# yanx27/PointASNL

Hardware: AMD Instinct MI355X
Metric: point-clouds/sec fwd (Bx1024 pts, ModelNet40 cls) (higher is better)
Workload: dtype f32; 1 GPU; configs[1]: ModelNet40 pointasnl_cls, 1024 pts, batch=64/GPU, seeded random weights; global_batch=64, parallelism=batch-shard x1, RCCL all-gather of logits, pipeline=prefetch, hip_graph=True, prefix_forked_at=start, prefix_levels=2, settle_replays=40, hip_hw_queues=4

## Files before the change

### include/pasnl.h

```cpp
#ifndef PASNL_H_
#define PASNL_H_

#include <stddef.h>
#include <stdint.h>

#ifdef __cplusplus
extern "C" {
#endif

#define PASNL_VERSION 100

enum {
  PASNL_OK = 0,
  PASNL_EINVAL = -1,
  PASNL_ENULL = -2,
  PASNL_EWORKSPACE = -3,
  PASNL_ELAUNCH = -4,
  PASNL_EUNSUPPORTED = -5
};

typedef void* pasnl_stream_t;

int pasnl_version(void);
const char* pasnl_strerror(int code);
// ... 90 lines not shown
                          const float* ww, const float* bw, float* out, float* skip_max, float* new_xyz, float* new_feature,
                          pasnl_stream_t stream);

int pasnl_sa_project(int b, int n, int c, int c1, const float* xyz, const float* feature, const float* w0, const float* b0,
                     float* proj, pasnl_stream_t stream);
int pasnl_sa_cell_pre(int b, int n, int c, int m, int k, int c1, int c2, const float* xyz, const float* feature,
                      const float* proj, const int* idx, const float* new_xyz, const float* w0, const float* w1, const float* b1,
                      const float* ww, const float* bw, float* out, float* skip_max, pasnl_stream_t stream);
int pasnl_sa_cell_pre_centre0(int b, int n, int c, int m, int k, int c1, int c2, const float* xyz, const float* feature,
                              const float* proj, const int* idx, const float* w0, const float* w1, const float* b1,
                              const float* ww, const float* bw, float* out, float* skip_max, float* new_xyz, float* new_feature,
                              pasnl_stream_t stream);

int pasnl_sa_cell_packed(int b, int n, int c, int npoint, int nsample, int c1, int c2, const float* xyz, const float* feature,
                         const int* idx, const float* new_xyz, const float* w0, const float* b0, const float* w1, const float* b1,
                         const float* ww, const float* bw, const float* w0_features_packed, const float* w1_packed, float* out,
                         float* skip_max, float* new_xyz_out, float* new_feature_out, pasnl_stream_t stream);

int pasnl_max_pool_rows(int b, int n, int c, const float* x, float* out, pasnl_stream_t stream);

int pasnl_max_pool_rows_strided(int b, int n, int c, const float* x, float* out, long out_stride, pasnl_stream_t stream);

size_t pasnl_mlp3_packed_weights_bytes(int k, int n);
int pasnl_mlp3_pack_weights(int k, int n, const float* w, float* packed, pasnl_stream_t stream);
size_t pasnl_mlp3_max_pool_workspace_bytes(int b, int n, int c3);
int pasnl_mlp3_max_pool(int b, int n, int k0, int c1, int c2, int c3, const float* x, const float* w0, const float* b0,
                        const float* w1, const float* b1, const float* w2, const float* b2, float* out, long out_stride,
                        void* workspace, size_t workspace_bytes, pasnl_stream_t stream);

int pasnl_cls_tail_group_all(int b, int n, int w, int cb, int c, const float* after, const float* skip_max, const float* att,
                             const float* ws_packed, const float* bs, const float* wb_packed, const float* bb,
                             const float* wagg_packed, const float* bagg, const float* new_xyz, int c1, int c2, int c3,
                             const float* w0, const float* b0, const float* w1, const float* b1, const float* w2, const float* b2,
                             float* out, float* pooled, long pooled_stride, void* workspace, size_t workspace_bytes,
                             pasnl_stream_t stream);

size_t pasnl_bf16x3_weights_bytes(int kdim, int n);
int pasnl_bf16x3_split_weights(int kdim, int n, const float* w, void* wsplit, pasnl_stream_t stream);
int pasnl_dense_bf16x3(int rows, int kdim, int n, int lda, const float* x, const void* wsplit, const float* bias, int relu,
                       float* out, pasnl_stream_t stream);


size_t pasnl_dense_rows_workspace_bytes(int rows, int kdim, int n);
int pasnl_dense_rows(int rows, int kdim, int n, const float* x, const float* w, const float* bias, int relu, float* out,
                     void* workspace, size_t workspace_bytes, pasnl_stream_t stream);

size_t pasnl_dense_splitk_workspace_bytes(int rows, int kdim, int n);
int pasnl_dense_splitk(int rows, int kdim, int n, int lda, const float* x, const float* w, const float* bias, int relu,
                       float* out, void* workspace, size_t workspace_bytes, pasnl_stream_t stream);

int pasnl_narrow_project2(long rows0, int kdim0, int n0, const float* x0, const float* w0, const float* bias0, float* out0,
                          long rows1, int kdim1, int n1, const float* x1, const float* w1, const float* bias1, float* out1,
                          pasnl_stream_t stream);

size_t pasnl_grad_workspace_bytes(int b, int targets, long contributions);
int pasnl_gather_point_grad_det(int b, int n, int m, const float* out_g, const int* idx, float* inp_g, void* workspace,
                                size_t workspace_bytes, pasnl_stream_t stream);
int pasnl_group_point_grad_det(int b, int n, int c, int m, int nsample, const float* grad_out, const int* idx,
                               float* grad_points, void* workspace, size_t workspace_bytes, pasnl_stream_t stream);
int pasnl_three_interpolate_grad_det(int b, int n, int c, int m, const float* grad_out, const int* idx, const float* weight,
                                     float* grad_points, void* workspace, size_t workspace_bytes, pasnl_stream_t stream);

int pasnl_sa_tail(int rows, int w, int cb, int c, const float* after, const float* skip_max, const float* att, const float* ws,
                  const float* bs, const float* wb, const float* bb, const float* wagg, const float* bagg, float* out,
                  pasnl_stream_t stream);

int pasnl_sa_tail_res(int rows, int w, int cb, int c, const float* after, const float* skip_max, const float* att,
                      const float* ws, const float* bs, const float* wb, const float* bb, const float* wagg,
                      const float* bagg, const float* residual, float* out, pasnl_stream_t stream);

size_t pasnl_sa_tail_packed_weights_bytes(int k, int c);
int pasnl_sa_tail_pack_weights(int k, int c, const float* w, float* packed, pasnl_stream_t stream);
int pasnl_sa_tail_packed(int rows, int w, int cb, int c, const float* after, const float* skip_max, const float* att,
                         const float* ws_packed, const float* bs, const float* wb_packed, const float* bb, const float* wagg_packed,
                         const float* bagg, const float* residual, const float* new_xyz, float* out_cat, float* out,
                         pasnl_stream_t stream);

int pasnl_sa_tail_cat(int rows, int w, int cb, int c, const float* after, const float* skip_max, const float* att,
                      const float* ws, const float* bs, const float* wb, const float* bb, const float* wagg,
                      const float* bagg, float* out, const float* new_xyz, float* out_cat, pasnl_stream_t stream);

int pasnl_decode_cell(int b, int n, int c, int k, const float* xyz, const float* feature, const int* idx, const float* ww,
                      const float* bw, float* out, pasnl_stream_t stream);

int pasnl_decode_cell_tiled(int b, int n, int c, int k, const float* xyz, const float* feature, const int* idx,
                            const float* ww, const float* bw, float* out, pasnl_stream_t stream);
int pasnl_decode_cell_tiled_v4(int c, const float* feature);

int pasnl_take_neighbor0(int b, int n, int c, int m, int k, const float* xyz, const float* feature, const int* idx,
                         float* new_xyz, float* new_feature, pasnl_stream_t stream);

int pasnl_as_gather(int b, int n, int c, int m, int k, int as, const float* xyz, const float* feature, const int* idx, float* out,
                    pasnl_stream_t stream);
int pasnl_as_attention_qkv(int g, int as, int cb, const float* kvq, float* out, pasnl_stream_t stream);
int pasnl_as_attention_proj(int g, int as, int cb, int w, const float* x, const float* wkvq, const float* bkvq, float* out,
                            pasnl_stream_t stream);
int pasnl_as_cell_narrow(int g, int as, int cb, int w, int ch, const float* x, const float* wkvq, const float* bkvq,
                         const float* wa, const float* ba, const float* wb, const float* bb, float* new_xyz, float* new_feature,
                         pasnl_stream_t stream);
int pasnl_as_cell_wide(int g, int as, int cb, int w, int ch, const float* kvq, const float* x, const float* wa, const float* ba,
                       const float* wb, const float* bb, float* new_xyz, float* new_feature, pasnl_stream_t stream);

int pasnl_as_cell_wide_ld(int g, int as, int cb, int w, int ch, const float* kvq, int ld, const float* x, const float* wa,
                          const float* ba, const float* wb, const float* bb, float* new_xyz, float* new_feature,
                          pasnl_stream_t stream);
int pasnl_as_reweight_x(int g, int as, int ch, const float* logits, const float* x, float* new_xyz, float* new_feature,
// ... 223 lines not shown
```

### pointasnl_amd/_hip.py

```python
import ctypes
import os

import torch

_HERE = os.path.dirname(os.path.abspath(__file__))
LIB_PATH = os.path.join(_HERE, "csrc", "libpasnl_hip.so")

SYMBOLS = [
    "pasnl_version", "pasnl_strerror", "pasnl_device_count",
    "pasnl_farthest_point_sample", "pasnl_farthest_point_sample_gather", "pasnl_gather_point", "pasnl_gather_point_grad", "pasnl_prob_sample",
    "pasnl_query_ball_point", "pasnl_sa_group", "pasnl_group_point", "pasnl_group_point_grad", "pasnl_select_top_k", "pasnl_knn_batch", "pasnl_knn_workspace_bytes", "pasnl_knn_batch_ws", "pasnl_knn_batch_ws_bg", "pasnl_knn_tree_workspace_bytes", "pasnl_knn_batch_tree", "pasnl_knn_batch_ref_workspace_bytes", "pasnl_knn_batch_ref", "pasnl_knn_distance_pick",
    "pasnl_three_nn", "pasnl_three_interpolate", "pasnl_three_interpolate_grad", "pasnl_three_weights", "pasnl_fp_interpolate_cat",
    "pasnl_nl_attention", "pasnl_nl_attention_workspace_bytes", "pasnl_nl_attention_ws", "pasnl_as_attention", "pasnl_as_reweight", "pasnl_sa_local_cell", "pasnl_sa_cell", "pasnl_sa_cell_centre0", "pasnl_sa_cell_packed", "pasnl_sa_project", "pasnl_sa_cell_pre", "pasnl_sa_cell_pre_centre0", "pasnl_sa_tail", "pasnl_sa_tail_cat", "pasnl_sa_tail_res", "pasnl_sa_tail_packed_weights_bytes", "pasnl_sa_tail_pack_weights", "pasnl_sa_tail_packed", "pasnl_decode_cell", "pasnl_decode_cell_tiled", "pasnl_decode_cell_tiled_v4", "pasnl_max_pool_rows", "pasnl_max_pool_rows_strided", "pasnl_mlp3_max_pool_workspace_bytes", "pasnl_mlp3_max_pool", "pasnl_mlp3_packed_weights_bytes", "pasnl_mlp3_pack_weights", "pasnl_dense_rows_workspace_bytes", "pasnl_dense_rows", "pasnl_dense_splitk_workspace_bytes", "pasnl_dense_splitk", "pasnl_bf16x3_weights_bytes", "pasnl_bf16x3_split_weights", "pasnl_dense_bf16x3", "pasnl_narrow_project2", "pasnl_take_neighbor0", "pasnl_as_gather", "pasnl_as_attention_qkv", "pasnl_as_attention_proj", "pasnl_as_cell_narrow", "pasnl_as_cell_wide", "pasnl_as_cell_wide_ld", "pasnl_as_reweight_x", "pasnl_grid_subsample_workspace_bytes", "pasnl_grid_subsample", "pasnl_knn_crop_workspace_bytes", "pasnl_knn_crop",
    "pasnl_scan_pick", "pasnl_knn_crop_indirect", "pasnl_crop_order_permute", "pasnl_scan_possibility_update", "pasnl_scan_scratch_init", "pasnl_scan_vote", "pasnl_scan_reproject_workspace_bytes", "pasnl_scan_reproject", "pasnl_scan_labels",
    "pasnl_scan_pick_given", "pasnl_scan_train_labels", "pasnl_scan_augment",
    "pasnl_scan_radius_workspace_bytes", "pasnl_scan_radius_members", "pasnl_scene_radius_members", "pasnl_scan_radius_gather", "pasnl_scene_radius_gather",
    "pasnl_scene_pick", "pasnl_knn_crop_scene", "pasnl_scene_pick_crop", "pasnl_scene_order_gather", "pasnl_scene_potential_update", "pasnl_scene_vote", "pasnl_scene_labels", "pasnl_confusion_matrix",
    "pasnl_window_noise", "pasnl_window_bounds", "pasnl_window_hist_bytes", "pasnl_window_count", "pasnl_window_fill", "pasnl_window_gather", "pasnl_window_vote", "pasnl_window_pool_labels",
    "pasnl_kwindow_hist_bytes", "pasnl_kwindow_count", "pasnl_kwindow_fill", "pasnl_kwindow_gather",
    "pasnl_modelnet_fps_cap", "pasnl_modelnet_fps", "pasnl_modelnet_normalize", "pasnl_modelnet_batch", "pasnl_modelnet_augment", "pasnl_modelnet_noise", "pasnl_cls_vote", "pasnl_cls_tally",
    "pasnl_cls_tail_group_all",
    "pasnl_block_key_capacity", "pasnl_block_crop_stats", "pasnl_block_grid_count", "pasnl_block_fill", "pasnl_block_gather", "pasnl_block_normalize", "pasnl_block_score_workspace_bytes", "pasnl_block_score", "pasnl_block_train_batch", "pasnl_block_train_score",
    "pasnl_kblock_crop_stats", "pasnl_kblock_grid_count", "pasnl_kblock_fill", "pasnl_kblock_gather", "pasnl_kblock_rotate",
    "pasnl_grad_workspace_bytes", "pasnl_gather_point_grad_det", "pasnl_group_point_grad_det", "pasnl_three_interpolate_grad_det",
]


class PasnlError(RuntimeError):
    pass


class PasnlUnsupported(PasnlError):
    """PASNL_EUNSUPPORTED: a valid request outside what the fused kernel covers (include/pasnl.h documents the limits).
    The cells catch it and take their op-by-op path (still HIP kernels + vendor GEMMs, never a CPU path)."""


_lib = None


def lib():
    global _lib
    if _lib is None:
        if not os.path.exists(LIB_PATH):
            raise PasnlError(
                f"{LIB_PATH} is missing: build it with `python -c 'import __graft_entry__ as g; g.build()'` "
                "(or `make -C pointasnl_amd/csrc`).  pointasnl_amd has no CPU or eager fallback.")
        _lib = ctypes.CDLL(LIB_PATH)
        _lib.pasnl_strerror.restype = ctypes.c_char_p
        _lib.pasnl_grad_workspace_bytes.restype = ctypes.c_size_t
        _lib.pasnl_knn_workspace_bytes.restype = ctypes.c_size_t
        _lib.pasnl_knn_tree_workspace_bytes.restype = ctypes.c_size_t
        _lib.pasnl_knn_batch_ref_workspace_bytes.restype = ctypes.c_size_t
        _lib.pasnl_dense_rows_workspace_bytes.restype = ctypes.c_size_t
        _lib.pasnl_bf16x3_weights_bytes.restype = ctypes.c_size_t
        _lib.pasnl_mlp3_max_pool_workspace_bytes.restype = ctypes.c_size_t
        _lib.pasnl_mlp3_packed_weights_bytes.restype = ctypes.c_size_t
        _lib.pasnl_sa_tail_packed_weights_bytes.restype = ctypes.c_size_t
        _lib.pasnl_dense_splitk_workspace_bytes.restype = ctypes.c_size_t
        _lib.pasnl_grid_subsample_workspace_bytes.restype = ctypes.c_size_t
        _lib.pasnl_knn_crop_workspace_bytes.restype = ctypes.c_size_t
        _lib.pasnl_scan_reproject_workspace_bytes.restype = ctypes.c_size_t
        _lib.pasnl_scan_radius_workspace_bytes.restype = ctypes.c_size_t
        _lib.pasnl_nl_attention_workspace_bytes.restype = ctypes.c_size_t
        _lib.pasnl_window_hist_bytes.restype = ctypes.c_size_t
        _lib.pasnl_kwindow_hist_bytes.restype = ctypes.c_size_t
        _lib.pasnl_block_score_workspace_bytes.restype = ctypes.c_size_t
        for s in SYMBOLS:
            getattr(_lib, s)
    return _lib


def require_device():
    if not torch.cuda.is_available():
        raise PasnlError("no HIP device visible: pointasnl_amd runs on MI355X (gfx950) only and has no CPU fallback")
# ... 99 lines not shown
```

### pointasnl_amd/models/pointasnl_cls.py

```python
import torch

from pointasnl_amd.utils import tf_util, pointasnl_util
from pointasnl_amd.utils.pointnet_util import pointnet_sa_module
from pointasnl_amd.utils.pointasnl_util import PointASNLSetAbstraction, get_repulsion_loss, sa_search, Forked


def first_layer(num_point=None):
    return dict(npoint=512, nsample=32)


def get_model(point_cloud, is_training=False, use_normal=False, bn_decay=None, weight_decay=None, num_class=40,
              adaptive_sample=False, search=None, before_head=None, fork_at="head", lazy_fork=None):
    if lazy_fork is None:
        lazy_fork = not adaptive_sample
    batch_size = point_cloud.shape[0]
    end_points = {}
    if use_normal:
        l0_xyz = point_cloud[:, :, 0:3].contiguous()
        l0_points = point_cloud[:, :, 3:6].contiguous()
    else:
        l0_xyz = point_cloud
        l0_points = point_cloud
    end_points['l0_xyz'] = l0_xyz
    as_neighbor = [12, 12] if adaptive_sample else [0, 0]

    net = torch.empty((batch_size, 1024 + 512), dtype=torch.float32, device=point_cloud.device)
    fuse3_1 = not adaptive_sample or pointasnl_util.SA_TAIL_GROUP_ALL == "always"

    search2 = []
    if isinstance(search, dict):
        search2.append(search[2])
        search = search[1]
    l1_xyz, l1_points = PointASNLSetAbstraction(l0_xyz, l0_points, npoint=512, nsample=32, mlp=[64, 64, 128],
                                                is_training=is_training, bn_decay=bn_decay, weight_decay=weight_decay,
                                                scope='layer1', as_neighbor=as_neighbor[0], search=search, xyz_concat=True,
                                                group_all=dict(mlp=[128, 256, 512], scope='layer3_1', pooled_out=net[:, 1024:]) if fuse3_1 else None,
                                                after_sampling=None if search2 else lambda xyz1: search2.append(
                                                    Forked(lambda: sa_search(xyz1, None, 128, 64), lazy=lazy_fork)))
    end_points['l1_xyz'] = l1_xyz
    l2_xyz, l2_points = PointASNLSetAbstraction(l1_xyz, l1_points, npoint=128, nsample=64, mlp=[128, 128, 256],
                                                is_training=is_training, bn_decay=bn_decay, weight_decay=weight_decay,
                                                scope='layer2', as_neighbor=as_neighbor[1], search=search2[0], xyz_concat=True,
                                                after_cell=before_head if fork_at == "cell2" else None,
                                                before_after_conv=before_head if fork_at == "conv2" else None)
    end_points['l2_xyz'] = l1_xyz
    if before_head is not None and fork_at == "head":
        before_head()
    if getattr(l1_points, "group_all_pooled", None) is None:
        _, l3_points_res, _ = pointnet_sa_module(l1_xyz, l1_points, npoint=None, radius=None, nsample=None,
                                                 mlp=[128, 256, 512], mlp2=None, group_all=True, is_training=is_training,
                                                 bn_decay=bn_decay, scope='layer3_1', pooled_out=net[:, 1024:])
    _, l3_points, _ = pointnet_sa_module(l2_xyz, l2_points, npoint=None, radius=None, nsample=None,
                                         mlp=[256, 512, 1024], mlp2=None, group_all=True, is_training=is_training,
                                         bn_decay=bn_decay, scope='layer3_2', pooled_out=net[:, :1024])

    net = tf_util.fully_connected(net, 512, bn=True, is_training=is_training, scope='fc1', bn_decay=bn_decay)
    net = tf_util.dropout(net, keep_prob=0.4, is_training=is_training, scope='dp1')
    net = tf_util.fully_connected(net, 256, bn=True, is_training=is_training, scope='fc2', bn_decay=bn_decay)
    net = tf_util.dropout(net, keep_prob=0.4, is_training=is_training, scope='dp2')
    net = tf_util.fully_connected(net, num_class, activation_fn=None, scope='fc3')
    end_points['l1_points'] = l1_points
    end_points['l2_points'] = l2_points
    end_points['l2_xyz_true'] = l2_xyz
    return net, end_points


def get_loss(pred, label, end_points, uniform_weight=0, weights_decay=1e-4):
    regularization_loss = tf_util.regularization_loss(weights_decay)
    loss = torch.nn.functional.cross_entropy(pred, label.long(), reduction='none')
    classify_loss = loss.mean()
    if uniform_weight > 0:
        uniform_loss = get_repulsion_loss(end_points['l1_xyz'], nsample=20, radius=0.07)
    else:
        uniform_loss = classify_loss
    return classify_loss + uniform_weight * uniform_loss + regularization_loss
```

### pointasnl_amd/utils/pointasnl_util.py

```python

import ctypes

import torch

from pointasnl_amd import _hip
from pointasnl_amd import tf_sampling, tf_grouping, nearest_neighbors
from pointasnl_amd.tf_interpolate import three_nn, three_interpolate, three_weights, fp_interpolate_cat
from pointasnl_amd.utils import tf_util, pointnet_util

NL_KEY_PARTS = True
NL_VARIANT = 0


KNN_TIE_ORDER = "reference"


def knn_query(k, support_pts, query_pts, out=None, max_workgroups=None):
    return nearest_neighbors.knn_batch(support_pts, query_pts, k, omp=True, dtype=torch.int32, tie_order=KNN_TIE_ORDER, out=out,
                                       max_workgroups=max_workgroups)


def _gather_rows(points, idx):
    return tf_grouping.group_point(points, idx.unsqueeze(-1)).squeeze(2)

# ... 302 lines not shown
            with tf_util.variable_scope('mlp2_1'):
                wb, bb = st.layer(32, 1 + channel, bn, weight_decay)
            ld = (3 * cb + 31) // 32 * 32 if AS_PAD_PROJECTION else 3 * cb
            if ld != 3 * cb:
                pkey = key + "@ld%d" % ld
                if pkey not in st._folded:
                    st._folded[pkey] = (torch.cat([wkvq, wkvq.new_zeros((6 + c, ld - 3 * cb))], dim=1).contiguous(),
                                        torch.cat([bkvq, bkvq.new_zeros(ld - 3 * cb)]).contiguous())
                wkvq, bkvq = st._folded[pkey]
            kvq = torch.addmm(bkvq, x.reshape(-1, 6 + c), wkvq)
            new_xyz = torch.empty((b, p, 3), dtype=torch.float32, device=xyz.device)
            new_feature = torch.empty((b, p, channel), dtype=torch.float32, device=xyz.device)
            _hip.launch("pasnl_as_cell_wide_ld", "as_cell", b * p, as_, cb, 6 + c, channel, _hip.ptr(kvq), int(ld), _hip.ptr(x),
                        _hip.ptr(wa), _hip.ptr(ba), _hip.ptr(wb), _hip.ptr(bb), _hip.ptr(new_xyz), _hip.ptr(new_feature))
            return new_xyz, new_feature
        att = torch.empty((b, p, as_, cb), dtype=torch.float32, device=xyz.device)
        if AS_PROJ_FUSED and 6 + c <= 15 and cb in (32, 64):
            _hip.launch("pasnl_as_attention_proj", "as_attention", b * p, as_, cb, 6 + c, _hip.ptr(x), _hip.ptr(wkvq),
                        _hip.ptr(bkvq), _hip.ptr(att))
        else:
            kvq = torch.addmm(bkvq, x.reshape(-1, 6 + c), wkvq)
            _hip.launch("pasnl_as_attention_qkv", "as_attention", b * p, as_, cb, _hip.ptr(kvq), _hip.ptr(att))
        hid = tf_util.conv2d(att, 32, [1, 1], padding='VALID', stride=[1, 1], bn=bn, is_training=False, scope='mlp2_0',
                             weight_decay=weight_decay)
        logits = tf_util.conv2d(hid, 1 + channel, [1, 1], padding='VALID', stride=[1, 1], bn=bn, is_training=False,
                                scope='mlp2_1', activation_fn=None, weight_decay=weight_decay).contiguous()
    new_xyz = torch.empty((b, p, 3), dtype=torch.float32, device=xyz.device)
    new_feature = torch.empty((b, p, channel), dtype=torch.float32, device=xyz.device)
    _hip.launch("pasnl_as_reweight_x", "as_reweight", b * p, as_, channel, _hip.ptr(logits), _hip.ptr(x), _hip.ptr(new_xyz),
                _hip.ptr(new_feature))
    return new_xyz, new_feature


def nl_attention(q, kv, variant=None):
    b, p, cb = q.shape
    n = kv.shape[1]
    q, kv = q.contiguous(), kv.contiguous()
    out = torch.empty_like(q)
    v = int(NL_VARIANT if variant is None else variant)
    nbytes = int(_hip.lib().pasnl_nl_attention_workspace_bytes(b, p, n, cb)) if v == 0 and NL_KEY_PARTS else 0
    if nbytes:
        ws = torch.empty((nbytes,), dtype=torch.uint8, device=q.device)
        _hip.launch("pasnl_nl_attention_ws", "nl_attention", b, p, n, cb, _hip.ptr(q), _hip.ptr(kv), _hip.ptr(out), v, _hip.ptr(ws),
                    ctypes.c_size_t(nbytes))
        return out
    _hip.launch("pasnl_nl_attention", "nl_attention", b, p, n, cb, _hip.ptr(q), _hip.ptr(kv), _hip.ptr(out), v)
    return out


AS_PAD_PROJECTION = True
XYZ_CONCAT = True
CENTRE0 = True
NL_NARROW_PROJECT = True


def PointNonLocalCell(feature, new_point, mlp, is_training, bn_decay, weight_decay, scope, bn=True, scaled=True,
                      mode='dot', project=True):
    if mode != 'dot' or not scaled:
        raise NotImplementedError("only mode='dot', scaled=True is reachable in the reference models (SURVEY a11)")
    with tf_util.variable_scope(scope):
        bottleneck_channel = mlp[0]
        batch_size, npoint, nsample, channel = new_point.shape
        if NL_NARROW_PROJECT and feature.shape[-1] <= 16 and channel <= 16 and bottleneck_channel in (32, 64, 128):
            tf_util._require_inference(is_training)
            st = tf_util.store()
            with tf_util.variable_scope('conv_kv'):
                wkv, bkv = st.layer(feature.shape[-1], 2 * bottleneck_channel, bn, weight_decay)
            with tf_util.variable_scope('conv_query'):
                wq, bq = st.layer(channel, bottleneck_channel, bn, weight_decay)
            n_all = feature.shape[1]
            feature, new_point = feature.contiguous(), new_point.contiguous()
            kv = torch.empty((batch_size, n_all, 2 * bottleneck_channel), dtype=torch.float32, device=feature.device)
            q = torch.empty((batch_size, npoint * nsample, bottleneck_channel), dtype=torch.float32, device=feature.device)
            _hip.launch("pasnl_narrow_project2", "narrow_project", ctypes.c_long(batch_size * n_all), int(feature.shape[-1]),
                        2 * bottleneck_channel, _hip.ptr(feature), _hip.ptr(wkv), _hip.ptr(bkv), _hip.ptr(kv),
                        ctypes.c_long(batch_size * npoint * nsample), int(channel), bottleneck_channel, _hip.ptr(new_point), _hip.ptr(wq),
                        _hip.ptr(bq), _hip.ptr(q))
            new_nonlocal_point = nl_attention(q, kv)
            if not project:
                return new_nonlocal_point
            new_nonlocal_point = tf_util.conv2d(
                new_nonlocal_point.reshape(batch_size, npoint, nsample, bottleneck_channel), mlp[-1], [1, 1],
                padding='VALID', stride=[1, 1], bn=bn, is_training=is_training, scope='conv_back_project',
                bn_decay=bn_decay, weight_decay=weight_decay)
            return new_nonlocal_point.squeeze(1)
        feature = feature.unsqueeze(2)
        transformed_feature = tf_util.conv2d(feature, bottleneck_channel * 2, [1, 1], padding='VALID', stride=[1, 1],
                                             bn=bn, is_training=is_training, scope='conv_kv', bn_decay=bn_decay,
                                             weight_decay=weight_decay, activation_fn=None)
        transformed_new_point = tf_util.conv2d(new_point, bottleneck_channel, [1, 1], padding='VALID', stride=[1, 1],
                                               bn=bn, is_training=is_training, scope='conv_query', bn_decay=bn_decay,
                                               weight_decay=weight_decay, activation_fn=None)
        transformed_new_point = transformed_new_point.reshape(batch_size, npoint * nsample, bottleneck_channel)
        try:
            new_nonlocal_point = nl_attention(transformed_new_point, transformed_feature.squeeze(2))
        except _hip.PasnlUnsupported:
            kv = transformed_feature.squeeze(2)
            attention_map = torch.matmul(transformed_new_point, kv[..., :bottleneck_channel].transpose(1, 2))
            attention_map = torch.softmax(attention_map / (float(bottleneck_channel) ** 0.5), dim=-1)
            new_nonlocal_point = torch.matmul(attention_map, kv[..., bottleneck_channel:])
        if not project:
            return new_nonlocal_point
        new_nonlocal_point = tf_util.conv2d(
            new_nonlocal_point.reshape(batch_size, npoint, nsample, bottleneck_channel), mlp[-1], [1, 1],
            padding='VALID', stride=[1, 1], bn=bn, is_training=is_training, scope='conv_back_project',
            bn_decay=bn_decay, weight_decay=weight_decay)
        new_nonlocal_point = new_nonlocal_point.squeeze(1)
        return new_nonlocal_point


import os as _os
OVERLAP = _os.environ.get("PASNL_OVERLAP", "1") != "0"
_SIDE_STREAMS = {}


def _side_stream(slot=0):
    key = (torch.cuda.current_device(), slot)
    if key not in _SIDE_STREAMS:
        _SIDE_STREAMS[key] = torch.cuda.Stream()
    return _SIDE_STREAMS[key]


LAZY_FORK = False


class Forked:

    def __init__(self, fn, slot=0, lazy=None):
        self.stream = None
        self._fn = None
        if not OVERLAP:
# ... 93 lines not shown

def sa_search(xyz, feature, npoint, nsample, use_knn=True, radius=None, knn_all=None):
    num_points = xyz.shape[1]
    if num_points == npoint:
        if knn_all is not None:
            k_all = _resolved(knn_all)
            idx = k_all if k_all.shape[2] == nsample else k_all[:, :, :nsample].contiguous()
        elif use_knn:
            idx = knn_query(nsample, xyz, xyz)
        else:
            idx, _ = tf_grouping.query_ball_point(radius, nsample, xyz, xyz)
        return xyz, None, idx
    if use_knn and knn_all is None and OVERLAP and SELF_KNN_RATIO * npoint >= num_points:
        knn_all = Forked(lambda: knn_query(nsample, xyz, xyz), slot=1)
    fps_idx, new_xyz = tf_sampling.farthest_point_sample_gather(npoint, xyz)
    if use_knn and knn_all is not None:
        k_all = _resolved(knn_all)
        idx = _gather_index_rows(k_all, fps_idx)
        if k_all.shape[2] != nsample:
            idx = idx[:, :, :nsample].contiguous()
    elif use_knn:
        idx = knn_query(nsample, xyz, new_xyz)
    else:
        idx, _ = tf_grouping.query_ball_point(radius, nsample, xyz, new_xyz)
    return new_xyz, None, idx


def sa_search_split(xyz, npoint, nsample, knn_all, slot=0):
    fp = Forked(lambda: tf_sampling.farthest_point_sample_gather(npoint, xyz), slot=slot)

    def join():
        fps_idx, new_xyz = fp.get()
        k_all = _resolved(knn_all)
        idx = _gather_index_rows(k_all, fps_idx)
        if k_all.shape[2] != nsample:
            idx = idx[:, :, :nsample].contiguous()
        return new_xyz, None, idx
    return Deferred(join)


def _tail_packed(st, w):
    key = "@tailpk:%x" % w.data_ptr()
    if key not in st._folded:
        wc = w.contiguous()
        pk = torch.empty(int(_hip.lib().pasnl_sa_tail_packed_weights_bytes(wc.shape[0], wc.shape[1])) // 4, dtype=torch.float32,
                         device=w.device)
        _hip.launch("pasnl_sa_tail_pack_weights", "sa_tail_pack", int(wc.shape[0]), int(wc.shape[1]), _hip.ptr(wc), _hip.ptr(pk))
        st._folded[key] = (pk, w)
    return st._folded[key][0]


def PointASNLSetAbstraction(xyz, feature, npoint, nsample, mlp, is_training, bn_decay, weight_decay, scope, bn=True,
                            use_knn=True, radius=None, as_neighbor=8, NL=True, search=None, after_sampling=None,
                            xyz_concat=False, after_cell=None, before_after_conv=None, residual=None, group_all=None):
    ga_weights = None
    if (group_all is not None and SA_TAIL_GROUP_ALL and SA_TAIL_FUSED and SA_TAIL_PACKED and NL and residual is None and not is_training
            and mlp[-1] == 128 and tuple(group_all['mlp']) == (128, 256, 512)):
        with tf_util.variable_scope(group_all['scope']):
            ga_weights = pointnet_util.group_all_weights(group_all['mlp'], 3 + mlp[-1], 1, bn)
    with tf_util.variable_scope(scope):
        batch_size, num_points, num_channel = feature.shape
        new_xyz, _, idx = _resolved(search) if search is not None else sa_search(xyz, feature, npoint, nsample, use_knn, radius)
        new_feature = feature
        nl_channel = mlp[-1]

        fused = _local_cell_supported(6 + num_channel, mlp, nsample)
        centre0 = False
        if num_points != npoint and as_neighbor == 0:
            xyz, feature, idx = xyz.contiguous(), feature.contiguous(), idx.contiguous()

            def take0():
                nx = torch.empty((batch_size, npoint, 3), dtype=torch.float32, device=xyz.device)
                nf = torch.empty((batch_size, npoint, 3 + num_channel), dtype=torch.float32, device=xyz.device)
                _hip.launch("pasnl_take_neighbor0", "take_neighbor0", batch_size, num_points, num_channel, npoint, nsample,
                            _hip.ptr(xyz), _hip.ptr(feature), _hip.ptr(idx), _hip.ptr(nx), _hip.ptr(nf))
                return nx, nf
            centre0 = (CENTRE0 and fused and SA_CELL_GATHER and npoint <= num_points
                       and (num_channel <= 128 or (SA_CELL_WIDE and mlp[0] in (256, 512) and nsample == 32)))
            if not centre0:
                new_xyz, new_feature = take0()
        elif num_points != npoint and AS_FUSED and as_neighbor <= 16:
            tf_util._require_inference(is_training)
            new_xyz, new_feature = adaptive_sampling_fused(xyz, feature, idx, as_neighbor, scope, bn, weight_decay)
        elif num_points != npoint:
            k_as = max(1, as_neighbor)
            idx_as = idx[:, :, :k_as].contiguous()
            g_xyz = tf_grouping.group_point(xyz, idx_as)
            g_pts = torch.cat([g_xyz, tf_grouping.group_point(feature, idx_as)], dim=-1)
            new_xyz, new_feature = AdaptiveSampling(g_xyz, g_pts, as_neighbor, is_training, bn_decay, weight_decay,
                                                    scope, bn)
        if after_sampling is not None and not centre0:
            after_sampling(new_xyz)
        new_point = None
        if fused and SA_CELL_GATHER:
            tf_util._require_inference(is_training)
            cell = sa_cell_pre if sa_cell_pre_supported(batch_size, num_points, num_channel, npoint, nsample, mlp, feature) else sa_cell
            try:
                if centre0:
                    new_point, skip_spatial, new_xyz, new_feature = cell(xyz, feature, idx, None, mlp, is_training,
                                                                         bn_decay, weight_decay, bn)
                else:
                    new_point, skip_spatial = cell(xyz, feature, idx, new_xyz, mlp, is_training, bn_decay, weight_decay, bn)
            except _hip.PasnlUnsupported:
                new_point = None
        if centre0:
            if new_point is None:
                new_xyz, new_feature = take0()
            if after_sampling is not None:
                after_sampling(new_xyz)
        if new_point is None:
            new_point, skip_spatial = sa_group(xyz, feature, idx, new_xyz)
            grouped_xyz = new_point[..., 0:3]
            if fused and not (len(mlp) == 3 and mlp[0] >= 32):
                fused = False
            if fused:
                tf_util._require_inference(is_training)
                try:
                    new_point = sa_local_cell(new_point, mlp, is_training, bn_decay, weight_decay, bn)
                except _hip.PasnlUnsupported:
                    fused = False
            if not fused:
                for i, num_out_channel in enumerate(mlp):
                    if i != len(mlp) - 1:
                        new_point = tf_util.conv2d(new_point, num_out_channel, [1, 1], padding='VALID', stride=[1, 1],
                                                   bn=bn, is_training=is_training, scope='conv%d' % (i),
                                                   bn_decay=bn_decay, weight_decay=weight_decay)
                weight = weight_net_hidden(grouped_xyz, [32], scope='weight_net', is_training=is_training,
                                           bn_decay=bn_decay, weight_decay=weight_decay)
                new_point = new_point.transpose(2, 3)
                new_point = torch.matmul(new_point, weight)

        if after_cell is not None:
            after_cell()
        c_out = mlp[-1]
        if SA_TAIL_FUSED and c_out % 32 == 0 and c_out <= 512 and batch_size * npoint >= SA_TAIL_MIN_ROWS:
            tf_util._require_inference(is_training)
            cb = max(32, num_channel // 2)
            att = None
            if NL:
                att = PointNonLocalCell(feature, new_feature.unsqueeze(1), [cb, nl_channel], is_training, bn_decay,
                                        weight_decay, scope, bn, project=False)
            if before_after_conv is not None:
                before_after_conv()
            after = tf_util.conv2d(new_point, c_out, [1, new_point.shape[2]], padding='VALID', stride=[1, 1], bn=bn,
                                   is_training=is_training, scope='after_conv', bn_decay=bn_decay, weight_decay=weight_decay)
            st = tf_util.store()
            w_in = skip_spatial.shape[-1]
            with tf_util.variable_scope('skip'):
                ws, bs = st.layer(w_in, c_out, bn, weight_decay)
            if NL:
                with tf_util.variable_scope(scope), tf_util.variable_scope('conv_back_project'):
                    wb, bb = st.layer(cb, c_out, bn, weight_decay)
            with tf_util.variable_scope('aggregation'):
                wagg, bagg = st.layer(c_out, c_out, bn, weight_decay)
            rows = batch_size * npoint
            after, skip_spatial = after.contiguous(), skip_spatial.contiguous()
            att = att.contiguous() if NL else None
            out = torch.empty((batch_size, npoint, c_out), dtype=torch.float32, device=xyz.device)
            args = (rows, int(w_in), int(cb if NL else 0), int(c_out), _hip.ptr(after), _hip.ptr(skip_spatial),
                    _hip.ptr(att), _hip.ptr(ws), _hip.ptr(bs), _hip.ptr(wb if NL else None),
                    _hip.ptr(bb if NL else None), _hip.ptr(wagg), _hip.ptr(bagg), _hip.ptr(out))
            try:
                if SA_TAIL_PACKED:
                    pk = [_tail_packed(st, m) if m is not None else None for m in (ws, wb if NL else None, wagg)]
                    cat = None
                    if ga_weights is not None and (int(w_in), int(cb)) == (9, 32) and new_xyz.shape[1] == npoint:
                        new_xyz = new_xyz.contiguous()
                        gmlp = group_all['mlp']
                        pooled = pointnet_util.group_all_pooled(group_all.get('pooled_out'), batch_size, gmlp[-1], xyz.device)
                        wsb = pointnet_util.group_all_workspace(batch_size, npoint, gmlp[-1], xyz.device)
                        _hip.launch("pasnl_cls_tail_group_all", "sa_tail_group_all", batch_size, npoint, int(w_in), int(cb), int(c_out),
                                    *args[4:7], _hip.ptr(pk[0]), args[8], _hip.ptr(pk[1]), args[10], _hip.ptr(pk[2]), args[12],
                                    _hip.ptr(new_xyz), gmlp[0], gmlp[1], gmlp[2], *[_hip.ptr(t) for t in ga_weights], args[13],
                                    _hip.ptr(pooled), ctypes.c_long(pooled.stride(0) if batch_size > 1 else gmlp[-1]),
                                    _hip.ptr(wsb), ctypes.c_size_t(wsb.numel()))
                        out.group_all_pooled = pooled
                        return new_xyz, out
                    if xyz_concat and XYZ_CONCAT:
                        new_xyz = new_xyz.contiguous()
                        cat = torch.empty((batch_size, npoint, 4 + c_out), dtype=torch.float32, device=xyz.device)
                    res_c = residual.contiguous() if residual is not None else None
                    _hip.launch("pasnl_sa_tail_packed", "sa_tail", *args[:7], _hip.ptr(pk[0]), args[8], _hip.ptr(pk[1]), args[10],
                                _hip.ptr(pk[2]), args[12], _hip.ptr(res_c), _hip.ptr(new_xyz if cat is not None else None),
                                _hip.ptr(cat), args[13])
                    residual = None
                    if cat is not None:
                        out.xyz_concat = (new_xyz, cat)
                elif residual is not None:
                    residual = residual.contiguous()
                    _hip.launch("pasnl_sa_tail_res", "sa_tail", *args[:-1], _hip.ptr(residual), args[-1])
                    residual = None
                elif xyz_concat and XYZ_CONCAT:
                    new_xyz = new_xyz.contiguous()
                    cat = torch.empty((batch_size, npoint, 4 + c_out), dtype=torch.float32, device=xyz.device)
                    _hip.launch("pasnl_sa_tail_cat", "sa_tail", *args, _hip.ptr(new_xyz), _hip.ptr(cat))
                    out.xyz_concat = (new_xyz, cat)
                else:
                    _hip.launch("pasnl_sa_tail", "sa_tail", *args)
            except _hip.PasnlUnsupported:
                tail = after.reshape(rows, c_out) + torch.relu_(torch.addmm(bs, skip_spatial.reshape(rows, w_in), ws))
                if NL:
                    tail = tail + torch.relu_(torch.addmm(bb, att.reshape(rows, cb), wb))
                out = torch.relu_(torch.addmm(bagg, tail, wagg)).reshape(batch_size, npoint, c_out)
            return new_xyz, (out if residual is None else out + residual)

        if NL:
            new_nonlocal_point = PointNonLocalCell(feature, new_feature.unsqueeze(1),
                                                   [max(32, num_channel // 2), nl_channel], is_training, bn_decay,
                                                   weight_decay, scope, bn)

        skip_spatial = tf_util.conv1d(skip_spatial, mlp[-1], 1, padding='VALID', stride=1, bn=bn,
                                      is_training=is_training, scope='skip', bn_decay=bn_decay,
                                      weight_decay=weight_decay)

        new_point = tf_util.conv2d(new_point, mlp[-1], [1, new_point.shape[2]], padding='VALID', stride=[1, 1], bn=bn,
                                   is_training=is_training, scope='after_conv', bn_decay=bn_decay,
                                   weight_decay=weight_decay)
        new_point = new_point.squeeze(2)
        new_point = new_point + skip_spatial
        if NL:
            new_point = new_point + new_nonlocal_point

        new_point = tf_util.conv1d(new_point, mlp[-1], 1, padding='VALID', stride=1, bn=bn, is_training=is_training,
                                   scope='aggregation', bn_decay=bn_decay, weight_decay=weight_decay)
        return new_xyz, (new_point if residual is None else new_point + residual)


DECODE_CELL_FUSED = True


DECODE_CELL_TILED = True
_DECODE_PERM = {}


def decode_tiled_order(c, v4, device):
    key = (c, bool(v4), str(device))
    if key not in _DECODE_PERM:
        V = 4 if v4 else 1
        T = torch.arange(c // 32).view(-1, 1, 1, 1, 1)
        g = torch.arange(4).view(1, -1, 1, 1, 1)
        h = torch.arange(2).view(1, 1, -1, 1, 1)
        m = torch.arange(32).view(1, 1, 1, -1, 1)
        i = torch.arange(4).view(1, 1, 1, 1, -1)
        ch = 3 + 32 * V * (T // V) + V * m + T % V
        j = 8 * g + 4 * h + i
        tiles = (ch * 32 + j).reshape(-1)
        _DECODE_PERM[key] = torch.cat([torch.arange(96), tiles]).to(device)
    return _DECODE_PERM[key]


def decode_cell(xyz, feature, idx, weight_decay=None):
    b, n, c = feature.shape
    k = idx.shape[2]
    with tf_util.variable_scope('decode_weight_net'), tf_util.variable_scope('wconv0'):
        ww, bw = tf_util.store().layer(3, 32, True, weight_decay)
    xyz, feature, idx = xyz.contiguous(), feature.contiguous(), idx.contiguous()
    out = torch.empty((b, n, 3 + c, 32), dtype=torch.float32, device=xyz.device)
    if DECODE_CELL_TILED and k == 16 and c % 32 == 0:
        v4 = int(_hip.lib().pasnl_decode_cell_tiled_v4(c, _hip.ptr(feature)))
        _hip.launch("pasnl_decode_cell_tiled", "decode_cell", b, n, c, k, _hip.ptr(xyz), _hip.ptr(feature), _hip.ptr(idx),
                    _hip.ptr(ww), _hip.ptr(bw), _hip.ptr(out))
        out.row_order = ("decode_tiled_c%d_v%d" % (c, v4), decode_tiled_order(c, v4, xyz.device))
# ... 65 lines not shown
```

Before: 56900 point-clouds/s.

## Compute first-layer non-local attention in input space with fused flash-style kernel

Adds a fused kernel for the first set-abstraction layer's non-local cell, used when the input feature width is at most 8 channels. The query is folded through the key projection into a tiny input-space vector. Online softmax then runs directly over the raw 3-channel points, and the value projection is applied to the weighted-mean point at the end. This avoids materialising the projected key/value and query tensors and the separate attention kernel, but it changes summation order, which can shift floating-point results slightly. A PasnlUnsupported fallback to the old projection-plus-attention path is kept.

```diff
diff --git a/include/pasnl.h b/include/pasnl.h
--- a/include/pasnl.h
+++ b/include/pasnl.h
@@ -166,6 +166,10 @@
 int pasnl_narrow_project2(long rows0, int kdim0, int n0, const float* x0, const float* w0, const float* bias0, float* out0,
                           long rows1, int kdim1, int n1, const float* x1, const float* w1, const float* bias1, float* out1,
                           pasnl_stream_t stream);
+
+int pasnl_cls_nl_cell_input(int b, int p, int n, int c, int cz, int cb, const float* feature, const float* new_point,
+                            const float* wkv, const float* bkv, const float* wq, const float* bq, float* out,
+                            pasnl_stream_t stream);
 
 size_t pasnl_grad_workspace_bytes(int b, int targets, long contributions);
 int pasnl_gather_point_grad_det(int b, int n, int m, const float* out_g, const int* idx, float* inp_g, void* workspace,
diff --git a/pointasnl_amd/_hip.py b/pointasnl_amd/_hip.py
--- a/pointasnl_amd/_hip.py
+++ b/pointasnl_amd/_hip.py
@@ -19,7 +19,7 @@
     "pasnl_window_noise", "pasnl_window_bounds", "pasnl_window_hist_bytes", "pasnl_window_count", "pasnl_window_fill", "pasnl_window_gather", "pasnl_window_vote", "pasnl_window_pool_labels",
     "pasnl_kwindow_hist_bytes", "pasnl_kwindow_count", "pasnl_kwindow_fill", "pasnl_kwindow_gather",
     "pasnl_modelnet_fps_cap", "pasnl_modelnet_fps", "pasnl_modelnet_normalize", "pasnl_modelnet_batch", "pasnl_modelnet_augment", "pasnl_modelnet_noise", "pasnl_cls_vote", "pasnl_cls_tally",
-    "pasnl_cls_tail_group_all",
+    "pasnl_cls_tail_group_all", "pasnl_cls_nl_cell_input",
     "pasnl_block_key_capacity", "pasnl_block_crop_stats", "pasnl_block_grid_count", "pasnl_block_fill", "pasnl_block_gather", "pasnl_block_normalize", "pasnl_block_score_workspace_bytes", "pasnl_block_score", "pasnl_block_train_batch", "pasnl_block_train_score",
     "pasnl_kblock_crop_stats", "pasnl_kblock_grid_count", "pasnl_kblock_fill", "pasnl_kblock_gather", "pasnl_kblock_rotate",
     "pasnl_grad_workspace_bytes", "pasnl_gather_point_grad_det", "pasnl_group_point_grad_det", "pasnl_three_interpolate_grad_det",
diff --git a/pointasnl_amd/csrc/nl_input.hip b/pointasnl_amd/csrc/nl_input.hip
--- /dev/null
+++ b/pointasnl_amd/csrc/nl_input.hip
@@ -0,0 +1,231 @@
+#include <math.h>
+#include "common.hpp"
+
+namespace pasnl {
+
+constexpr float NLI_LOG2E = 1.4426950408889634f;
+constexpr int NLI_KB = 16;
+constexpr int NLI_CHUNK = 256;
+constexpr int NLI_MIN_KEYS = 64;
+
+__device__ __forceinline__ float nli_exp2(float x) { return __builtin_amdgcn_exp2f(x); }
+
+template <int CT, int RW, bool MASK>
+__device__ __forceinline__ void nli_block(const float* rowp, int valid, const float (&u)[CT], float& m, float& l, float (&acc)[CT]) {
+  float x[NLI_KB][RW], s[NLI_KB];
+#pragma unroll
+  for (int j = 0; j < NLI_KB; ++j)
+#pragma unroll
+    for (int g = 0; g < RW / 4; ++g) {
+      const float4 v = *reinterpret_cast<const float4*>(rowp + j * RW + 4 * g);
+      x[j][4 * g] = v.x; x[j][4 * g + 1] = v.y; x[j][4 * g + 2] = v.z; x[j][4 * g + 3] = v.w;
+    }
+#pragma unroll
+  for (int j = 0; j < NLI_KB; ++j) {
+    float t = u[0] * x[j][0];
+#pragma unroll
+    for (int ch = 1; ch < CT; ++ch) t = fmaf(u[ch], x[j][ch], t);
+    s[j] = (MASK && j >= valid) ? -INFINITY : t;
+  }
+  float bm = s[0];
+#pragma unroll
+  for (int j = 1; j < NLI_KB; ++j) bm = fmaxf(bm, s[j]);
+  const float mnew = fmaxf(m, bm);
+  const float alpha = nli_exp2(m - mnew);
+  l *= alpha;
+#pragma unroll
+  for (int ch = 0; ch < CT; ++ch) acc[ch] *= alpha;
+#pragma unroll
+  for (int j = 0; j < NLI_KB; ++j) {
+    const float pj = nli_exp2(s[j] - mnew);
+    l += pj;
+#pragma unroll
+    for (int ch = 0; ch < CT; ++ch) acc[ch] = fmaf(pj, x[j][ch], acc[ch]);
+  }
+  m = mnew;
+}
+
+template <int CT, int SPLIT>
+__global__ __launch_bounds__(SPLIT * 64) void nl_input_kernel(int p, int n, int c, int cz, int cb, float scale,
+                                                              const float* __restrict__ feature,
+                                                              const float* __restrict__ new_point,
+                                                              const float* __restrict__ wkv, const float* __restrict__ bkv,
+                                                              const float* __restrict__ wq, const float* __restrict__ bq,
+                                                              float* __restrict__ out) {
+  constexpr int RW = CT <= 4 ? 4 : 8;
+  constexpr int WAVE_ROWS = NLI_CHUNK * RW;
+  constexpr int PARK = (CT + 2) * 64;
+  constexpr int RPL = NLI_CHUNK / 64;
+  extern __shared__ __align__(16) float nli_smem[];
+  const int lane = lane_id();
+  const int wave = __builtin_amdgcn_readfirstlane((int)(threadIdx.x >> 6));
+  float* rows = nli_smem + wave * WAVE_ROWS;
+  float* park = nli_smem + SPLIT * WAVE_ROWS;
+  const int bi = blockIdx.y, q0 = blockIdx.x * 64;
+  const int qi = min(q0 + lane, p - 1);
+  const float* zrow = new_point + ((size_t)bi * p + qi) * cz;
+  const float* f = feature + (size_t)bi * n * c;
+
+  float u[CT];
+#pragma unroll
+  for (int ch = 0; ch < CT; ++ch) u[ch] = 0.f;
+  for (int kg = wave * 4; kg < cb; kg += SPLIT * 4) {
+    float qv[4];
+#pragma unroll
+    for (int j = 0; j < 4; ++j) qv[j] = bq[kg + j];
+    for (int i = 0; i < cz; ++i) {
+      const float zi = zrow[i];
+#pragma unroll
+      for (int j = 0; j < 4; ++j) qv[j] = fmaf(zi, wq[i * cb + kg + j], qv[j]);
+    }
+#pragma unroll
+    for (int ch = 0; ch < CT; ++ch)
+      if (CT == 3 || ch < c) {
+#pragma unroll
+        for (int j = 0; j < 4; ++j) u[ch] = fmaf(qv[j], wkv[ch * 2 * cb + kg + j], u[ch]);
+      }
+  }
+#pragma unroll
+  for (int ch = 0; ch < CT; ++ch) park[wave * PARK + ch * 64 + lane] = u[ch];
+  __syncthreads();
+#pragma unroll
+  for (int ch = 0; ch < CT; ++ch) {
+    float t = park[ch * 64 + lane];
+    for (int w = 1; w < SPLIT; ++w) t += park[w * PARK + ch * 64 + lane];
+    u[ch] = t * scale;
+  }
+  __syncthreads();
+
+  const int per = ((n + SPLIT - 1) / SPLIT + NLI_KB - 1) / NLI_KB * NLI_KB;
+  const int k0 = (int)min((long)wave * per, (long)n), k1 = (int)min((long)k0 + per, (long)n);
+  float m = -INFINITY, l = 0.f, acc[CT];
+#pragma unroll
+  for (int ch = 0; ch < CT; ++ch) acc[ch] = 0.f;
+
+  float pre[RPL][CT];
+  auto fetch = [&](int kc) {
+#pragma unroll
+    for (int r = 0; r < RPL; ++r) {
+      const int key = kc + r * 64 + lane;
+#pragma unroll
+      for (int ch = 0; ch < CT; ++ch) pre[r][ch] = (key < k1 && (CT == 3 || ch < c)) ? f[(size_t)key * c + ch] : 0.f;
+    }
+  };
+  if (k0 < k1) fetch(k0);
+  for (int kc = k0; kc < k1; kc += NLI_CHUNK) {
+#pragma unroll
+    for (int r = 0; r < RPL; ++r)
+#pragma unroll
+      for (int g = 0; g < RW / 4; ++g) {
+        float4 v;
+        v.x = pre[r][4 * g];
+        v.y = 4 * g + 1 < CT ? pre[r][4 * g + 1 < CT ? 4 * g + 1 : 0] : 0.f;
+        v.z = 4 * g + 2 < CT ? pre[r][4 * g + 2 < CT ? 4 * g + 2 : 0] : 0.f;
+        v.w = 4 * g + 3 < CT ? pre[r][4 * g + 3 < CT ? 4 * g + 3 : 0] : 0.f;
+        *reinterpret_cast<float4*>(rows + (r * 64 + lane) * RW + 4 * g) = v;
+      }
+    __builtin_amdgcn_fence(__ATOMIC_RELEASE, "wavefront");
+    __builtin_amdgcn_wave_barrier();
+    __builtin_amdgcn_fence(__ATOMIC_ACQUIRE, "wavefront");
+    if (kc + NLI_CHUNK < k1) fetch(kc + NLI_CHUNK);
+    const int cnt = min(NLI_CHUNK, k1 - kc);
+    int j0 = 0;
+    for (; j0 + NLI_KB <= cnt; j0 += NLI_KB) nli_block<CT, RW, false>(rows + j0 * RW, NLI_KB, u, m, l, acc);
+    if (j0 < cnt) nli_block<CT, RW, true>(rows + j0 * RW, cnt - j0, u, m, l, acc);
+    __builtin_amdgcn_fence(__ATOMIC_RELEASE, "wavefront");
+    __builtin_amdgcn_wave_barrier();
+    __builtin_amdgcn_fence(__ATOMIC_ACQUIRE, "wavefront");
+  }
+
+  if (wave > 0) {
+#pragma unroll
+    for (int ch = 0; ch < CT; ++ch) park[wave * PARK + ch * 64 + lane] = acc[ch];
+    park[wave * PARK + CT * 64 + lane] = m;
+    park[wave * PARK + (CT + 1) * 64 + lane] = l;
+  }
+  __syncthreads();
+  if (wave == 0) {
+    for (int w = 1; w < SPLIT; ++w) {
+      const float* pw = park + w * PARK;
+      const float mw = pw[CT * 64 + lane], lw = pw[(CT + 1) * 64 + lane];
+      const float mnew = fmaxf(m, mw);
+      const float a0 = m == -INFINITY ? 0.f : nli_exp2(m - mnew);
+      const float a1 = mw == -INFINITY ? 0.f : nli_exp2(mw - mnew);
+      l = l * a0 + lw * a1;
+      m = mnew;
+#pragma unroll
+      for (int ch = 0; ch < CT; ++ch) acc[ch] = acc[ch] * a0 + pw[ch * 64 + lane] * a1;
+    }
+    const float inv = 1.0f / l;
+#pragma unroll
+    for (int ch = 0; ch < CT; ++ch) park[ch * 64 + lane] = acc[ch] * inv;
+  }
+  __syncthreads();
+  float ctr[CT];
+#pragma unroll
+  for (int ch = 0; ch < CT; ++ch) ctr[ch] = park[ch * 64 + lane];
+  if (q0 + lane < p) {
+    float* op = out + ((size_t)bi * p + q0 + lane) * cb;
+    for (int kg = wave * 4; kg < cb; kg += SPLIT * 4) {
+      float o[4];
+#pragma unroll
+      for (int j = 0; j < 4; ++j) o[j] = bkv[cb + kg + j];
+#pragma unroll
+      for (int ch = 0; ch < CT; ++ch)
+        if (CT == 3 || ch < c) {
+#pragma unroll
+          for (int j = 0; j < 4; ++j) o[j] = fmaf(ctr[ch], wkv[ch * 2 * cb + cb + kg + j], o[j]);
+        }
+      *reinterpret_cast<float4*>(op + kg) = make_float4(o[0], o[1], o[2], o[3]);
+    }
+  }
+}
+
+template <int CT, int SPLIT>
+static int nl_input_launch(int b, int p, int n, int c, int cz, int cb, float scale, const float* feature, const float* new_point,
+                    const float* wkv, const float* bkv, const float* wq, const float* bq, float* out, hipStream_t st) {
+  const size_t lds = (size_t)SPLIT * (NLI_CHUNK * (CT <= 4 ? 4 : 8) + (CT + 2) * 64) * sizeof(float);
+  if (launch(nl_input_kernel<CT, SPLIT>, dim3((p + 63) / 64, b), dim3(SPLIT * 64), lds, st, p, n, c, cz, cb, scale, feature,
+             new_point, wkv, bkv, wq, bq, out) != PASNL_OK)
+    return PASNL_ELAUNCH;
+  return pasnl_launch_status();
+}
+
+static int nl_input_split(int b, int p, int n) {
+  const long tiles = (long)b * ((p + 63) / 64);
+  int split = 4;
+  while (split < 16 && tiles * split < 2048 && n / (split * 2) >= NLI_MIN_KEYS) split *= 2;
+  return split;
+}
+
+template <int CT>
+static int nl_input_dispatch(int b, int p, int n, int c, int cz, int cb, float scale, const float* feature, const float* new_point,
+                      const float* wkv, const float* bkv, const float* wq, const float* bq, float* out, hipStream_t st) {
+  const int split = nl_input_split(b, p, n);
+  if constexpr (CT <= 4) {
+    if (split == 16) return nl_input_launch<CT, 16>(b, p, n, c, cz, cb, scale, feature, new_point, wkv, bkv, wq, bq, out, st);
+  }
+  switch (split) {
+    case 16:
+    case 8: return nl_input_launch<CT, 8>(b, p, n, c, cz, cb, scale, feature, new_point, wkv, bkv, wq, bq, out, st);
+    default: return nl_input_launch<CT, 4>(b, p, n, c, cz, cb, scale, feature, new_point, wkv, bkv, wq, bq, out, st);
+  }
+}
+
+}
+
+extern "C" int pasnl_cls_nl_cell_input(int b, int p, int n, int c, int cz, int cb, const float* feature, const float* new_point,
+                                       const float* wkv, const float* bkv, const float* wq, const float* bq, float* out,
+                                       pasnl_stream_t stream) {
+  using namespace pasnl;
+  PASNL_REQUIRE(b >= 0 && p >= 0 && n >= 1 && c >= 1 && cz >= 1 && cb >= 1, PASNL_EINVAL);
+  PASNL_REQUIRE(c <= 8 && cz <= 16 && (cb == 32 || cb == 64 || cb == 128), PASNL_EUNSUPPORTED);
+  if (b == 0 || p == 0) return PASNL_OK;
+  PASNL_REQUIRE(feature && new_point && wkv && bkv && wq && bq && out, PASNL_ENULL);
+  PASNL_REQUIRE(b <= 65535, PASNL_EUNSUPPORTED);
+  PASNL_REQUIRE((reinterpret_cast<uintptr_t>(out) & 15) == 0, PASNL_EUNSUPPORTED);
+  hipStream_t st = pasnl_hip_stream(stream);
+  const float scale = NLI_LOG2E / sqrtf((float)cb);
+  if (c == 3) return nl_input_dispatch<3>(b, p, n, c, cz, cb, scale, feature, new_point, wkv, bkv, wq, bq, out, st);
+  return nl_input_dispatch<8>(b, p, n, c, cz, cb, scale, feature, new_point, wkv, bkv, wq, bq, out, st);
+}
diff --git a/pointasnl_amd/models/pointasnl_cls.py b/pointasnl_amd/models/pointasnl_cls.py
--- a/pointasnl_amd/models/pointasnl_cls.py
+++ b/pointasnl_amd/models/pointasnl_cls.py
@@ -26,6 +26,7 @@
 
     net = torch.empty((batch_size, 1024 + 512), dtype=torch.float32, device=point_cloud.device)
     fuse3_1 = not adaptive_sample or pointasnl_util.SA_TAIL_GROUP_ALL == "always"
+    nl_input_space = not adaptive_sample or pointasnl_util.NL_INPUT_SPACE == "always"
 
     search2 = []
     if isinstance(search, dict):
@@ -34,6 +35,7 @@
     l1_xyz, l1_points = PointASNLSetAbstraction(l0_xyz, l0_points, npoint=512, nsample=32, mlp=[64, 64, 128],
                                                 is_training=is_training, bn_decay=bn_decay, weight_decay=weight_decay,
                                                 scope='layer1', as_neighbor=as_neighbor[0], search=search, xyz_concat=True,
+                                                nl_input_space=nl_input_space,
                                                 group_all=dict(mlp=[128, 256, 512], scope='layer3_1', pooled_out=net[:, 1024:]) if fuse3_1 else None,
                                                 after_sampling=None if search2 else lambda xyz1: search2.append(
                                                     Forked(lambda: sa_search(xyz1, None, 128, 64), lazy=lazy_fork)))
diff --git a/pointasnl_amd/utils/pointasnl_util.py b/pointasnl_amd/utils/pointasnl_util.py
--- a/pointasnl_amd/utils/pointasnl_util.py
+++ b/pointasnl_amd/utils/pointasnl_util.py
@@ -378,10 +378,11 @@
 XYZ_CONCAT = True
 CENTRE0 = True
 NL_NARROW_PROJECT = True
+NL_INPUT_SPACE = True
 
 
 def PointNonLocalCell(feature, new_point, mlp, is_training, bn_decay, weight_decay, scope, bn=True, scaled=True,
-                      mode='dot', project=True):
+                      mode='dot', project=True, input_space=True):
     if mode != 'dot' or not scaled:
         raise NotImplementedError("only mode='dot', scaled=True is reachable in the reference models (SURVEY a11)")
     with tf_util.variable_scope(scope):
@@ -396,13 +397,24 @@
                 wq, bq = st.layer(channel, bottleneck_channel, bn, weight_decay)
             n_all = feature.shape[1]
             feature, new_point = feature.contiguous(), new_point.contiguous()
-            kv = torch.empty((batch_size, n_all, 2 * bottleneck_channel), dtype=torch.float32, device=feature.device)
-            q = torch.empty((batch_size, npoint * nsample, bottleneck_channel), dtype=torch.float32, device=feature.device)
-            _hip.launch("pasnl_narrow_project2", "narrow_project", ctypes.c_long(batch_size * n_all), int(feature.shape[-1]),
-                        2 * bottleneck_channel, _hip.ptr(feature), _hip.ptr(wkv), _hip.ptr(bkv), _hip.ptr(kv),
-                        ctypes.c_long(batch_size * npoint * nsample), int(channel), bottleneck_channel, _hip.ptr(new_point), _hip.ptr(wq),
-                        _hip.ptr(bq), _hip.ptr(q))
-            new_nonlocal_point = nl_attention(q, kv)
+            new_nonlocal_point = None
+            if NL_INPUT_SPACE and input_space and feature.shape[-1] <= 8:
+                att = torch.empty((batch_size, npoint * nsample, bottleneck_channel), dtype=torch.float32, device=feature.device)
+                try:
+                    _hip.launch("pasnl_cls_nl_cell_input", "nl_cell_input", batch_size, npoint * nsample, int(n_all),
+                                int(feature.shape[-1]), int(channel), bottleneck_channel, _hip.ptr(feature), _hip.ptr(new_point),
+                                _hip.ptr(wkv), _hip.ptr(bkv), _hip.ptr(wq), _hip.ptr(bq), _hip.ptr(att))
+                    new_nonlocal_point = att
+                except _hip.PasnlUnsupported:
+                    pass
+            if new_nonlocal_point is None:
+                kv = torch.empty((batch_size, n_all, 2 * bottleneck_channel), dtype=torch.float32, device=feature.device)
+                q = torch.empty((batch_size, npoint * nsample, bottleneck_channel), dtype=torch.float32, device=feature.device)
+                _hip.launch("pasnl_narrow_project2", "narrow_project", ctypes.c_long(batch_size * n_all), int(feature.shape[-1]),
+                            2 * bottleneck_channel, _hip.ptr(feature), _hip.ptr(wkv), _hip.ptr(bkv), _hip.ptr(kv),
+                            ctypes.c_long(batch_size * npoint * nsample), int(channel), bottleneck_channel, _hip.ptr(new_point),
+                            _hip.ptr(wq), _hip.ptr(bq), _hip.ptr(q))
+                new_nonlocal_point = nl_attention(q, kv)
             if not project:
                 return new_nonlocal_point
             new_nonlocal_point = tf_util.conv2d(
@@ -602,7 +614,8 @@
 
 def PointASNLSetAbstraction(xyz, feature, npoint, nsample, mlp, is_training, bn_decay, weight_decay, scope, bn=True,
                             use_knn=True, radius=None, as_neighbor=8, NL=True, search=None, after_sampling=None,
-                            xyz_concat=False, after_cell=None, before_after_conv=None, residual=None, group_all=None):
+                            xyz_concat=False, after_cell=None, before_after_conv=None, residual=None, group_all=None,
+                            nl_input_space=True):
     ga_weights = None
     if (group_all is not None and SA_TAIL_GROUP_ALL and SA_TAIL_FUSED and SA_TAIL_PACKED and NL and residual is None and not is_training
             and mlp[-1] == 128 and tuple(group_all['mlp']) == (128, 256, 512)):
@@ -689,7 +702,7 @@
             att = None
             if NL:
                 att = PointNonLocalCell(feature, new_feature.unsqueeze(1), [cb, nl_channel], is_training, bn_decay,
-                                        weight_decay, scope, bn, project=False)
+                                        weight_decay, scope, bn, project=False, input_space=nl_input_space)
             if before_after_conv is not None:
                 before_after_conv()
             after = tf_util.conv2d(new_point, c_out, [1, new_point.shape[2]], padding='VALID', stride=[1, 1], bn=bn,
@@ -757,7 +770,7 @@
         if NL:
             new_nonlocal_point = PointNonLocalCell(feature, new_feature.unsqueeze(1),
                                                    [max(32, num_channel // 2), nl_channel], is_training, bn_decay,
-                                                   weight_decay, scope, bn)
+                                                   weight_decay, scope, bn, input_space=nl_input_space)
 
         skip_spatial = tf_util.conv1d(skip_spatial, mlp[-1], 1, padding='VALID', stride=1, bn=bn,
                                       is_training=is_training, scope='skip', bn_decay=bn_decay,
```

Result: faster. 58510 point-clouds/s, median of 6 (+2.8%).
